# grantjr1842/delayed-streams-modeling

Hardware: AMD Instinct MI355X
Metric: real-time stream throughput, stt-1b-en_fr @ bs=64 per GPU (Mimi encode + LM decode per 80 ms frame) (higher is better)
Workload: dtype bf16 weights + bf16 KV, f32 activations as three exact bf16 pieces, f32 accumulate (v_mfma_f32_16x16x32_bf16); 1 GPU; stt-1b-en_fr batch=64 streaming, ring KV cache full (750 frames), Mimi encode + LM decode HIP path; streams_per_gpu=64, parallelism=replicas x1 (independent stream batches, no per-step collective), streams=encoder stream || 2 LM group stream(s)

## Files before the change

### delayed-streams-modeling_amd/csrc/dsm_engine_api.inc

```

namespace {

template <typename KVT, int HD, int T>
int launch_attn_t(DsmDevice* e, hipStream_t st, float* out, const float* q, const void* k, const void* v,
                  const uint32_t* start_pos, const uint8_t* active, int B, int H, int ctx, int d, const AttnFused& fq) {
  constexpr int UNR = (sizeof(KVT) == 2 && T == 1 && HD == 128) ? 8 : 4;
  size_t lds = sizeof(float) * ((size_t)T * ctx + 4 * T * HD + 16);
  if ((long)B * H >= 2048 && (size_t)2 * ctx * HD * sizeof(KVT) >= (size_t)256 * 1024) lds += e->attn_lds_pad;
  if (lds > 64 * 1024) {
    static size_t allowed = 0;
    if (lds > allowed) {
      HIPCHK(hipFuncSetAttribute(reinterpret_cast<const void*>(&attn_kernel<KVT, HD, T, UNR>), hipFuncAttributeMaxDynamicSharedMemorySize, (int)lds));
      allowed = lds;
    }
  }
  const int tag = e->tag_attn[e->sid(st)];
  if (T == 1 && HD == 64 && ctx <= 32) {
    const int ph = e->prof_begin(tag, st);
    hipLaunchKernelGGL((attn_small_kernel<KVT, 64>), dim3((B * H + 3) / 4), dim3(256), 0, st, out, q, reinterpret_cast<const KVT*>(k),
                       reinterpret_cast<const KVT*>(v), start_pos, active, B * H, H, ctx, d, fq);
    e->prof_end(ph, st);
    HIPCHK(hipGetLastError());
    return 0;
  }
  const int ph = e->prof_begin(tag, st);
  hipLaunchKernelGGL((attn_kernel<KVT, HD, T, UNR>), dim3(B * H), dim3(256), lds, st, out, q, reinterpret_cast<const KVT*>(k),
                     reinterpret_cast<const KVT*>(v), start_pos, active, H, ctx, d, e->dev_ts_slot(tag, e->sid(st), 0), fq);
  e->prof_end(ph, st);
  HIPCHK(hipGetLastError());
  return 0;
}

template <typename KVT>
int launch_attn(DsmDevice* e, hipStream_t st, float* out, const float* q, const void* k, const void* v,
                const uint32_t* start_pos, const uint8_t* active, int B, int H, int hd, int T, int ctx, int d,
                const AttnFused& fq) {
#define DSM_ATTN(HDv, Tv) \
  if (hd == HDv && T == Tv) return launch_attn_t<KVT, HDv, Tv>(e, st, out, q, k, v, start_pos, active, B, H, ctx, d, fq);
  DSM_ATTN(32, 1) DSM_ATTN(64, 1) DSM_ATTN(128, 1) DSM_ATTN(32, 2) DSM_ATTN(64, 2) DSM_ATTN(128, 2)
#undef DSM_ATTN
  e->set_error("unsupported attention shape head_dim=%d T=%d (head_dim must be 32, 64 or 128; T 1 or 2)", hd, T);
  return DSM_ERR_INVALID;
}

int run_norm(DsmDevice* e, hipStream_t st, float* y, const float* x, const float* w, const float* b, int rows, int d,
             int rms) {
  hipLaunchKernelGGL(row_norm_kernel, dim3(rows), dim3(256), 0, st, y, x, w, b, rows, d,
                     rms ? 1e-8f : 1e-5f, rms);
  HIPCHK(hipGetLastError());
  return 0;
}

template <typename WT, typename KVT>
int transformer_forward(DsmDevice* e, hipStream_t st, const TransformerW& w, TransformerState& s, float* x, float* xn,
                        float* q, float* att, float* ff, int B, int T, const uint8_t* d_mask, float* final_out,
                        RowMap final_map, const float* post_norm_w = nullptr, float* post_norm_out = nullptr, int phase = 0,
                        const CaState* ca = nullptr, bool head_done = false) {
  const dsm_transformer_config& c = w.cfg;
  const int d = c.d_model, H = c.num_heads, hd = d / H, M = B * T;
  const float eps = c.norm == 1 ? 1e-8f : 1e-5f;
  if (phase != 2 && !head_done) {
    hipLaunchKernelGGL(kv_builder_kernel, dim3(B), dim3(64), 0, st, s.pos, s.idx, d_mask, s.start_pos, s.widx,
                       c.positional_embedding == 1 ? s.rope_cs : (float*)nullptr, w.inv_freq, B, T, c.context, hd,
                       w.rope_pos_before ? 1 : 0);
    HIPCHK(hipGetLastError());
    if (int rc = run_norm(e, st, xn, x, w.layers[0].n1w, w.layers[0].n1b, M, d, c.norm)) return rc;
  }
  for (int l = 0; l < c.num_layers; ++l) {
    const TLayerW& L = w.layers[l];
    const bool last = (l == c.num_layers - 1);
    AttnFused fq{};
    fq.nt = sizeof(KVT) == 2;
    if (!(phase == 2 && l == 0)) {
      GemmArgs a = base_args(L.in_proj, xn, plain_map(M, d), M);
      a.Y = q;
      a.d = d; a.hd = hd; a.H = H; a.T = T; a.ctx = c.context;
      a.kcache = s.k[l]; a.vcache = s.v[l];
      a.widx = s.widx;
      a.rope_cs = c.positional_embedding == 1 ? s.rope_cs : nullptr;
      a.active = d_mask;
      a.defer_reduce = (T == 1 && L.in_proj.Kpad > DSM_KC && L.in_proj.K % 32 == 0 && e->fuse_qkv) ? 1 : 0;
      if (int rc = launch_gemm_t<WT, KVT, EPI_QKV, 1>(e, st, a, true)) return rc;
      if (a.defer_reduce) {
        const int mtiles = (M + 15) / 16;
        fq.ws = a.ws;
        fq.ld = (long)a.ws_ntiles * 16;
        fq.cstride = (long)mtiles * 16 * fq.ld;
        fq.chunks = (a.Kpad + DSM_KC - 1) / DSM_KC;
        fq.rope_cs = a.rope_cs;
        fq.widx = s.widx;
      }
    }
    if (!(phase == 2 && l == 0))
      if (int rc = launch_attn<KVT>(e, st, att, q, s.k[l], s.v[l], s.start_pos, d_mask, B, H, hd, T, c.context, d, fq)) return rc;
    if (phase == 1) return 0;
    {
      GemmArgs a = base_args(L.out_proj, att, plain_map(M, d), M);
      a.scale = L.ls1;
      a.res = x; a.rmap = plain_map(M, d);
      a.Y = x; a.ymap = plain_map(M, d);
      if (ca) {
        a.norm_w = L.ncw; a.norm_b = L.ncb; a.norm_out = xn; a.norm_eps = w.ca_norm_rms ? 1e-8f : 1e-5f; a.norm_rms = w.ca_norm_rms;
      } else {
        a.norm_w = L.n2w; a.norm_b = L.n2b; a.norm_out = xn; a.norm_eps = eps; a.norm_rms = c.norm;
      }
      if (int rc = gemm_store<WT>(e, st, a)) return rc;
    }
    if (ca) {
      AttnFused none{};
      none.nt = fq.nt;
      {
        GemmArgs a = base_args(L.ca_q, xn, plain_map(M, d), M);
        a.Y = q; a.ymap = plain_map(M, d);
        a.defer_reduce = (T == 1 && a.Kpad > DSM_KC && a.K % 32 == 0 && !a.bias && d % 4 == 0 && e->fuse_qkv) ? 1 : 0;
        if (int rc = gemm_store<WT>(e, st, a)) return rc;
        if (a.defer_reduce) {
          none.ws = a.ws;
          none.ld = (long)a.ws_ntiles * 16;
          none.cstride = (long)((M + 15) / 16) * 16 * none.ld;
          none.chunks = (a.Kpad + DSM_KC - 1) / DSM_KC;
          none.q_only = 1;
        }
      }
      if (int rc = launch_attn<KVT>(e, st, ca->att, q, ca->k[l], ca->v[l], ca->last, ca->act, B, H, hd, T, ca->smax, d, none)) return rc;
      GemmArgs a = base_args(L.ca_out, ca->att, plain_map(M, d), M);
      a.res = x; a.rmap = plain_map(M, d);
      a.Y = x; a.ymap = plain_map(M, d);
      a.norm_w = L.n2w; a.norm_b = L.n2b; a.norm_out = xn; a.norm_eps = eps; a.norm_rms = c.norm;
      if (int rc = gemm_store<WT>(e, st, a)) return rc;
    }
    if (c.gating) {
      GemmArgs a = base_args(L.ff_in, xn, plain_map(M, d), M);
      a.N = w.hidden;
      a.nt_stride = w.hidden;
      a.Y = ff; a.ymap = plain_map(M, w.hidden);
      if (int rc = launch_gemm_t<WT, KVT, EPI_GATE, 2>(e, st, a, true)) return rc;
    } else {
      GemmArgs a = base_args(L.ff_in, xn, plain_map(M, d), M);
      a.act = 1;
      a.Y = ff; a.ymap = plain_map(M, w.hidden);
      if (int rc = gemm_store<WT>(e, st, a)) return rc;
    }
    {
      GemmArgs a = base_args(L.ff_out, ff, plain_map(M, w.hidden), M);
      a.scale = L.ls2;
      a.res = x; a.rmap = plain_map(M, d);
      if (last && final_out) {
        a.Y = final_out; a.ymap = final_map;
      } else {
        a.Y = x; a.ymap = plain_map(M, d);
      }
      if (!last) {
        a.norm_w = w.layers[l + 1].n1w; a.norm_b = w.layers[l + 1].n1b; a.norm_out = xn; a.norm_eps = eps; a.norm_rms = c.norm;
      } else if (post_norm_out) {
        a.norm_w = post_norm_w; a.norm_b = nullptr; a.norm_out = post_norm_out; a.norm_eps = eps; a.norm_rms = c.norm;
      }
      if (int rc = gemm_store<WT>(e, st, a)) return rc;
    }
  }
  return 0;
}

template <typename F>
int with_kv_type(bool kv_bf16, F&& f) {
  return kv_bf16 ? f(uint16_t{}) : f(float{});
}

int fork_groups(DsmDevice* e, hipStream_t st, size_t G) {
  if (G > 1) {
    HIPCHK(hipEventRecord(e->ev_fork, st));
    for (size_t g = 1; g < G; ++g) HIPCHK(hipStreamWaitEvent(e->s_grp[g], e->ev_fork, 0));
  }
  return 0;
}
template <typename F>
int run_groups(DsmDevice* e, hipStream_t st, size_t G, bool serialize, F&& body) {
  for (size_t g = G; g-- > 0;) {
    hipStream_t gs = (g == 0 || serialize) ? st : e->s_grp[g];
    if (int rc = body(g, gs)) return rc;
    if (g > 0) HIPCHK(hipEventRecord(e->ev_grp_done[g], gs));
  }
  return 0;
}
int join_groups(DsmDevice* e, hipStream_t st, size_t G) {
  for (size_t g = 1; g < G; ++g) HIPCHK(hipStreamWaitEvent(st, e->ev_grp_done[g], 0));
  return 0;
}

int mimi_encode_body(dsm_engine* e, int side, hipStream_t st);
int mimi_encode(dsm_engine* e, int side, hipStream_t st) {
  return run_captured(e, *e->g_enc[side], st, (uint64_t)e->sid(st), [&] { return mimi_encode_body(e, side, st); });
}
int mimi_encode_body(dsm_engine* e, int side, hipStream_t st) {
  const MimiW& w = e->mimi_w;
  MimiState& s = e->mimi[side];
  const int B = e->B;
  const RowMap none = plain_map(1, 1);
  e->tag_gemm[e->sid(st)] = DSM_PROF_GEMM_MIMI;
  e->tag_attn[e->sid(st)] = DSM_PROF_ATTN_MIMI;
  bool fused_front = false;
  {
    const MimiW::Stage& s0 = w.stages[0];
    const ConvGeom& c = w.init_conv;
    fused_front = e->fuse_front && c.in_c == 1 && c.k == 7 && c.stride == 1 && c.out_c == 64 && c.S == 6 && !c.lin.bf16 &&
                  s0.ra.k == 3 && s0.ra.stride == 1 && s0.ra.in_c == 64 && s0.ra.out_c == 32 && s0.ra.S == 2 && !s0.ra.lin.bf16 &&
                  s0.rb.k == 1 && s0.rb.stride == 1 && s0.rb.in_c == 32 && s0.rb.out_c == 64 && !s0.rb.lin.bf16 &&
                  c.T_in % 64 == 0 && c.T_out == c.T_in && s0.ra.T_in == c.T_in && s0.rb.T_in == c.T_in && s0.down.in_c == 64 &&
                  s0.down.T_in == c.T_in && !c.replicate && !s0.ra.replicate;
    if (fused_front) {
      SeanetFrontArgs fa;
      fa.cat_init = s.cat_init;
      fa.w0 = reinterpret_cast<const float*>(c.lin.w); fa.b0 = c.lin.bias; fa.ld0 = c.lin.Kpad;
      fa.w1 = reinterpret_cast<const float*>(s0.ra.lin.w); fa.b1 = s0.ra.lin.bias; fa.ld1 = s0.ra.lin.Kpad;
      fa.w2 = reinterpret_cast<const float*>(s0.rb.lin.w); fa.b2 = s0.rb.lin.bias; fa.ld2 = s0.rb.lin.Kpad;
      fa.cat_ra = s.stages[0].cat_ra;
      fa.cat_down = s.stages[0].cat_down;
      fa.T = c.T_in; fa.S0 = c.S; fa.Sd = s0.down.S;
      const int ph = e->prof_begin(e->tag_gemm[e->sid(st)], st);
      hipLaunchKernelGGL(seanet_front_kernel<64>, dim3(c.T_in / 64, B), dim3(256), seanet_front_lds<64>(), st, fa);
      e->prof_end(ph, st);
      HIPCHK(hipGetLastError());
    } else if (int rc = run_conv(e, st, c, s.cat_init, B, s.stages[0].y, plain_map(B * c.T_out, c.out_c), s.stages[0].cat_ra,
                                 cat_map(s0.ra), nullptr, none)) {
      return rc;
    }
  }
  for (size_t i = 0; i < w.stages.size(); ++i) {
    const MimiW::Stage& sw = w.stages[i];
    MimiState::Stage& ss = s.stages[i];
    if (!(i == 0 && fused_front)) {
      if (int rc = run_conv(e, st, sw.ra, ss.cat_ra, B, nullptr, none, ss.cat_rb, cat_map(sw.rb), nullptr, none)) return rc;
      if (int rc = run_conv(e, st, sw.rb, ss.cat_rb, B, nullptr, none, ss.cat_down, cat_map(sw.down), ss.y,
                            plain_map(B * sw.rb.T_out, sw.rb.out_c)))
        return rc;
    }
    if (i + 1 < w.stages.size()) {
      const MimiW::Stage& nx = w.stages[i + 1];
      if (int rc = run_conv(e, st, sw.down, ss.cat_down, B, s.stages[i + 1].y,
                            plain_map(B * sw.down.T_out, sw.down.out_c), s.stages[i + 1].cat_ra, cat_map(nx.ra), nullptr, none))
        return rc;
    } else {
      if (int rc = run_conv(e, st, sw.down, ss.cat_down, B, nullptr, none, s.cat_final, cat_map(w.final_conv), nullptr, none))
        return rc;
    }
  }
  const int Tt = w.final_conv.T_out, d = w.cfg.dimension;
  if (int rc = run_conv(e, st, w.final_conv, s.cat_final, B, s.x_tr, plain_map(B * Tt, d), nullptr, none, nullptr, none))
    return rc;
  if (int rc = transformer_forward<float, float>(e, st, w.tr, s.tr, s.x_tr, s.xn, s.q, s.att, s.ff, B, Tt, s.mask,
                                                  s.cat_ds, cat_map(w.downsample)))
    return rc;
  if (s.first_call && w.downsample.S > 0) {
    hipLaunchKernelGGL(conv_replicate_init_kernel, dim3(B), dim3(256), 0, st, s.h_descs[s.ds_desc]);
    HIPCHK(hipGetLastError());
  }
  if (int rc = run_conv(e, st, w.downsample, s.cat_ds, B, s.latent, plain_map(B, d), nullptr, none, nullptr, none)) return rc;
  const int n_q = w.cfg.quantizer_n_q, qd = w.cfg.quantizer_dim;
  e->tag_gemm[e->sid(st)] = DSM_PROF_RVQ;
  for (int which = 0; which < 2; ++which) {
    const RvqW& r = which == 0 ? w.rvq_first : w.rvq_rest;
    if (r.n_q == 0) continue;
    float* res = which == 0 ? s.res_first : s.res_rest;
    {
// ... 1185 lines not shown
```

### delayed-streams-modeling_amd/csrc/dsm_kernels.h

```cpp
#pragma once
#include <hip/hip_runtime.h>
#include <stdint.h>
#include "dsm_numerics.h"
#include "dsm_sampling.h"

typedef float f32x4 __attribute__((ext_vector_type(4)));
typedef short dsm_bf16x8 __attribute__((ext_vector_type(8)));

__device__ __forceinline__ float wave_sum64(float v) {
#pragma unroll
  for (int off = 32; off >= 1; off >>= 1) v = v + __shfl_xor(v, off, 64);
  return v;
}

enum { EPI_STORE = 0, EPI_QKV = 1, EPI_GATE = 2, EPI_RVQ = 3 };

struct RowMap {
  long bstride;
  int rpb;
  int ld;
  int toff;
  __host__ __device__ long off(int m) const { return (long)(m / rpb) * bstride + (long)((m % rpb) + toff) * ld; }
};

struct GemmArgs {
  const float* X;
  RowMap xmap;
  const void* W;
  int Kpad, K, N, M;
  int nt_stride;
  int wpacked;
  int w_ntiles;
  int wg_cols;
  const float* bias;
  const float* scale;
  const float* res;
  RowMap rmap;
  float* Y;
  RowMap ymap;
  float* Y2;
  RowMap y2map;
  int act;
  int vec;
  int d, hd, H, T, ctx;
  void* kcache;
  void* vcache;
  const uint32_t* widx;
  const float* rope_cs;
  const uint8_t* active;
  float* pval;
  uint32_t* pidx;
  float* ws;
  int ws_ntiles;
  int defer_reduce;
  int chunk_loop;
  const float* norm_w;
  const float* norm_b;
  float* norm_out;
  float norm_eps;
  int norm_rms;
  unsigned long long* ts;
};

template <typename WT>
__device__ __forceinline__ const WT* dsm_wbase(const GemmArgs& a, const WT* W, int n0, int r, int q) {
  if (sizeof(WT) == 2 && a.wpacked) return W + ((long)(n0 >> 4) * (a.Kpad >> 5)) * 512 + (q * 16 + r) * 8;
  return W + (long)(n0 + r) * a.Kpad + 8 * q;
}
template <typename WT>
__device__ __forceinline__ int dsm_wstep(const GemmArgs& a) { return (sizeof(WT) == 2 && a.wpacked) ? 16 : 1; }

__device__ __forceinline__ void launch_stamp_begin(unsigned long long* ts) {
  if (!ts || threadIdx.x != 0) return;
  const unsigned lin = blockIdx.x + gridDim.x * (blockIdx.y + gridDim.y * blockIdx.z);
  if (lin < 128) atomicMin(&ts[0], wall_clock64());
}
__device__ __forceinline__ void launch_stamp_end(unsigned long long* ts) {
  if (!ts || threadIdx.x != 0) return;
  const unsigned total = gridDim.x * gridDim.y * gridDim.z;
  const unsigned lin = blockIdx.x + gridDim.x * (blockIdx.y + gridDim.y * blockIdx.z);
  if (lin + 512 >= total) atomicMax(&ts[1], wall_clock64());
}

template <typename WT>
__device__ __forceinline__ void load_w8(const WT* p, float (&o)[8]);
template <>
__device__ __forceinline__ void load_w8<uint16_t>(const uint16_t* p, float (&o)[8]) {
  uint4 v = *reinterpret_cast<const uint4*>(p);
  o[0] = __uint_as_float(v.x << 16); o[1] = __uint_as_float(v.x & 0xFFFF0000u);
  o[2] = __uint_as_float(v.y << 16); o[3] = __uint_as_float(v.y & 0xFFFF0000u);
  o[4] = __uint_as_float(v.z << 16); o[5] = __uint_as_float(v.z & 0xFFFF0000u);
  o[6] = __uint_as_float(v.w << 16); o[7] = __uint_as_float(v.w & 0xFFFF0000u);
}
template <>
__device__ __forceinline__ void load_w8<float>(const float* p, float (&o)[8]) {
  float4 a = *reinterpret_cast<const float4*>(p);
  float4 b = *reinterpret_cast<const float4*>(p + 4);
  o[0] = a.x; o[1] = a.y; o[2] = a.z; o[3] = a.w; o[4] = b.x; o[5] = b.y; o[6] = b.z; o[7] = b.w;
}

template <typename KVT>
struct Raw8;
typedef unsigned int dsm_u32x4 __attribute__((ext_vector_type(4)));
typedef float dsm_f32x4v __attribute__((ext_vector_type(4)));
template <>
struct Raw8<uint16_t> {
  uint4 v;
  __device__ __forceinline__ void load(const uint16_t* p) { v = *reinterpret_cast<const uint4*>(p); }
  __device__ __forceinline__ void load_nt(const uint16_t* p) {
    const dsm_u32x4 t = __builtin_nontemporal_load(reinterpret_cast<const dsm_u32x4*>(p));
    v = make_uint4(t[0], t[1], t[2], t[3]);
  }
  __device__ __forceinline__ void unpack(float (&o)[8]) const {
    o[0] = __uint_as_float(v.x << 16); o[1] = __uint_as_float(v.x & 0xFFFF0000u);
    o[2] = __uint_as_float(v.y << 16); o[3] = __uint_as_float(v.y & 0xFFFF0000u);
    o[4] = __uint_as_float(v.z << 16); o[5] = __uint_as_float(v.z & 0xFFFF0000u);
    o[6] = __uint_as_float(v.w << 16); o[7] = __uint_as_float(v.w & 0xFFFF0000u);
  }
};
template <>
struct Raw8<float> {
  float4 a, b;
  __device__ __forceinline__ void load(const float* p) {
    a = *reinterpret_cast<const float4*>(p);
    b = *reinterpret_cast<const float4*>(p + 4);
  }
  __device__ __forceinline__ void load_nt(const float* p) {
    const dsm_f32x4v t0 = __builtin_nontemporal_load(reinterpret_cast<const dsm_f32x4v*>(p));
    const dsm_f32x4v t1 = __builtin_nontemporal_load(reinterpret_cast<const dsm_f32x4v*>(p + 4));
    a = make_float4(t0[0], t0[1], t0[2], t0[3]);
    b = make_float4(t1[0], t1[1], t1[2], t1[3]);
  }
  __device__ __forceinline__ void unpack(float (&o)[8]) const {
    o[0] = a.x; o[1] = a.y; o[2] = a.z; o[3] = a.w; o[4] = b.x; o[5] = b.y; o[6] = b.z; o[7] = b.w;
  }
};

__device__ __forceinline__ void store_kv(uint16_t* p, float v) { *p = dsm_f32_to_bf16(v); }
__device__ __forceinline__ void store_kv(float* p, float v) { *p = v; }

__device__ __forceinline__ void store_kv4(uint16_t* p, const float (&o)[4]) {
  uint2 v;
  v.x = (uint32_t)dsm_f32_to_bf16(o[0]) | ((uint32_t)dsm_f32_to_bf16(o[1]) << 16);
  v.y = (uint32_t)dsm_f32_to_bf16(o[2]) | ((uint32_t)dsm_f32_to_bf16(o[3]) << 16);
  *reinterpret_cast<uint2*>(p) = v;
}
__device__ __forceinline__ void store_kv4(float* p, const float (&o)[4]) {
  *reinterpret_cast<float4*>(p) = make_float4(o[0], o[1], o[2], o[3]);
}

template <typename KVT, int EPI>
__device__ __forceinline__ void epi_store_qkv(const GemmArgs& a, f32x4 v, int m, int n) {
  if (m >= a.M || n >= a.N) return;
  const bool full = a.vec && (n + 3 < a.N);
  if (EPI == EPI_STORE) {
    float o[4];
#pragma unroll
    for (int i = 0; i < 4; ++i) {
      float t = v[i];
      if (n + i < a.N) {
        if (a.bias) t = t + a.bias[n + i];
        if (a.act == 1) t = dsm_gelu_erf(t);
        if (a.scale) t = t * a.scale[n + i];
      }
      o[i] = t;
    }
    if (a.res) {
      const float* rp = a.res + a.rmap.off(m) + n;
      if (full) {
        float4 rv = *reinterpret_cast<const float4*>(rp);
        o[0] = rv.x + o[0]; o[1] = rv.y + o[1]; o[2] = rv.z + o[2]; o[3] = rv.w + o[3];
      } else {
#pragma unroll
        for (int i = 0; i < 4; ++i)
          if (n + i < a.N) o[i] = rp[i] + o[i];
      }
    }
    if (a.Y) {
      float* y = a.Y + a.ymap.off(m) + n;
      if (full) {
        *reinterpret_cast<float4*>(y) = make_float4(o[0], o[1], o[2], o[3]);
      } else {
#pragma unroll
        for (int i = 0; i < 4; ++i)
          if (n + i < a.N) y[i] = o[i];
      }
    }
    if (a.Y2) {
      float* y2 = a.Y2 + a.y2map.off(m) + n;
      if (full) {
        *reinterpret_cast<float4*>(y2) = make_float4(dsm_elu(o[0]), dsm_elu(o[1]), dsm_elu(o[2]), dsm_elu(o[3]));
      } else {
#pragma unroll
        for (int i = 0; i < 4; ++i)
          if (n + i < a.N) y2[i] = dsm_elu(o[i]);
      }
    }
  } else {
    const int part = n / a.d, c = n - part * a.d, h = c / a.hd, i0 = c - h * a.hd;
    const int b = m / a.T;
    float o[4] = {v[0], v[1], v[2], v[3]};
    if (part < 2 && a.rope_cs) {
      const float4 cs = *reinterpret_cast<const float4*>(a.rope_cs + ((long)m * (a.hd / 2) + (i0 >> 1)) * 2);
      const float co[2] = {cs.x, cs.z}, si[2] = {cs.y, cs.w};
#pragma unroll
      for (int p = 0; p < 2; ++p) {
        float x0 = v[2 * p], x1 = v[2 * p + 1];
        float t0 = x0 * co[p], t1 = x1 * si[p], t2 = x0 * si[p], t3 = x1 * co[p];
        o[2 * p] = t0 - t1;
        o[2 * p + 1] = t2 + t3;
      }
    }
    if (part == 0) {
      *reinterpret_cast<float4*>(a.Y + (long)m * a.d + c) = make_float4(o[0], o[1], o[2], o[3]);
    } else if (a.active[b]) {
      KVT* cache = reinterpret_cast<KVT*>(part == 1 ? a.kcache : a.vcache);
      store_kv4(cache + (((long)b * a.H + h) * a.ctx + a.widx[m]) * a.hd + i0, o);
    }
  }
}

__device__ __forceinline__ void epi_gate(const GemmArgs& a, f32x4 g, f32x4 u, int m, int n) {
  if (m >= a.M || n >= a.N) return;
  float o[4];
#pragma unroll
  for (int i = 0; i < 4; ++i) o[i] = dsm_silu(g[i]) * u[i];
  float* y = a.Y + a.ymap.off(m) + n;
  if (a.vec && n + 3 < a.N) {
    *reinterpret_cast<float4*>(y) = make_float4(o[0], o[1], o[2], o[3]);
  } else {
#pragma unroll
    for (int i = 0; i < 4; ++i)
      if (n + i < a.N) y[i] = o[i];
  }
}

__device__ __forceinline__ void epi_rvq(const GemmArgs& a, f32x4 v, int m, int n, int tile16, int q) {
  float bv = DSM_INF_F;
  uint32_t bi = 0xFFFFFFFFu;
#pragma unroll
  for (int i = 0; i < 4; ++i) {
    float dist = a.bias[n + i] - v[i];
    if (n + i < a.N && (dist < bv || (dist == bv && (uint32_t)(n + i) < bi))) { bv = dist; bi = (uint32_t)(n + i); }
  }
#pragma unroll
  for (int off = 16; off <= 32; off <<= 1) {
    float ov = __shfl_xor(bv, off, 64);
    uint32_t oi = __shfl_xor(bi, off, 64);
    if (ov < bv || (ov == bv && oi < bi)) { bv = ov; bi = oi; }
  }
  if (q == 0 && m < a.M) {
    a.pval[(long)tile16 * a.M + m] = bv;
    a.pidx[(long)tile16 * a.M + m] = bi;
  }
}

template <typename WT, typename KVT, int MT, int NT, int EPI, bool XALIGNED, bool BX3 = false>
__global__ void gemm_mfma_kernel(GemmArgs a) {
  extern __shared__ __attribute__((aligned(16))) float lds_part[];
  const int lane = threadIdx.x & 63, wave = threadIdx.x >> 6, S = blockDim.x >> 6;
  const int r = lane & 15, q = lane >> 4;
  const int m_base = blockIdx.y * (16 * MT);
  const int n_base = blockIdx.x * ((EPI == EPI_GATE) ? 16 : 16 * NT);
  const WT* W = reinterpret_cast<const WT*>(a.W);
  constexpr int TILES = NT * MT;

  const WT* wrow[NT];
#pragma unroll
  for (int nt = 0; nt < NT; ++nt) wrow[nt] = dsm_wbase<WT>(a, W, n_base + nt * a.nt_stride, r, q);
  const int wst = dsm_wstep<WT>(a);
  const float* xrow[MT];
#pragma unroll
  for (int mt = 0; mt < MT; ++mt) {
    int m = m_base + 16 * mt + r;
    m = m < a.M ? m : a.M - 1;
    xrow[mt] = a.X + a.xmap.off(m) + 8 * q;
  }
  f32x4 acc[NT][MT];
  const int chunks = (a.Kpad + DSM_KC - 1) / DSM_KC;

  for (int c = wave; c < chunks; c += S) {
#pragma unroll
    for (int nt = 0; nt < NT; ++nt)
#pragma unroll
      for (int mt = 0; mt < MT; ++mt) acc[nt][mt] = (f32x4){0.f, 0.f, 0.f, 0.f};
    const int k0 = c * DSM_KC;
    const int k1 = min(k0 + DSM_KC, a.Kpad);
    for (int kb = k0; kb < k1; kb += 32) {
      float wa[NT][8], xb[MT][8];
#pragma unroll
// ... 548 lines not shown
}

#define DSM_ROW_ITS 4

__device__ __forceinline__ void row_norm_apply(const float4 (&v)[DSM_ROW_ITS], float s, float s2, int d, float eps, int rms,
                                               const float* __restrict__ w, const float* __restrict__ b,
                                               float* __restrict__ out) {
  float mm = 1.f, mean = 0.f, inv = 0.f;
  if (rms) {
    mm = sqrtf(s2 / (float)d + eps);
  } else {
    mean = s / (float)d;
    float var = s2 / (float)d - mean * mean;
    inv = 1.0f / sqrtf(var + eps);
  }
#pragma unroll
  for (int it = 0; it < DSM_ROW_ITS; ++it) {
    const int i = it * 1024 + 4 * (int)threadIdx.x;
    if (i < d) {
      const float4 wv = *reinterpret_cast<const float4*>(w + i);
      float4 o;
      if (rms) {
        o.x = (v[it].x / mm) * wv.x; o.y = (v[it].y / mm) * wv.y; o.z = (v[it].z / mm) * wv.z; o.w = (v[it].w / mm) * wv.w;
      } else {
        const float4 bv = *reinterpret_cast<const float4*>(b + i);
        o.x = ((v[it].x - mean) * inv) * wv.x + bv.x; o.y = ((v[it].y - mean) * inv) * wv.y + bv.y;
        o.z = ((v[it].z - mean) * inv) * wv.z + bv.z; o.w = ((v[it].w - mean) * inv) * wv.w + bv.w;
      }
      *reinterpret_cast<float4*>(out + i) = o;
    }
  }
}

template <int ITS>
__global__ __launch_bounds__(256 * ITS) void gemm_reduce_rows_kernel(GemmArgs a, int chunks) {
  constexpr int RS = ITS == 4 ? 16 : 24;
  __shared__ float red[8];
  __shared__ float carry[2][256];
  launch_stamp_begin(a.ts ? a.ts + 2 : nullptr);
  const int m = blockIdx.x;
  const int d = a.N;
  const int it = threadIdx.x >> 8, t = threadIdx.x & 255;
  const long ld = (long)a.ws_ntiles * 16, cstride = (long)((a.M + 15) >> 4) * 16 * ld;
  const int i = it * 1024 + 4 * t;
  const bool live = i < d;
  const float* p = a.ws + (long)m * ld + (live ? i : 4 * t);
  const int ic = live ? i : 4 * t;
  const f32x4 bias4 = *reinterpret_cast<const f32x4*>(a.bias ? a.bias + ic : p);
  const f32x4 scale4 = *reinterpret_cast<const f32x4*>(a.scale ? a.scale + ic : p);
  const f32x4 res4 = *reinterpret_cast<const f32x4*>(a.res ? a.res + a.rmap.off(m) + ic : p);
  const f32x4 nw4 = *reinterpret_cast<const f32x4*>(a.norm_w + ic);
  const f32x4 nb4 = *reinterpret_cast<const f32x4*>(a.norm_rms ? p : a.norm_b + ic);
  f32x4 tot = *reinterpret_cast<const f32x4*>(p);
  for (int c0 = 1; c0 < chunks; c0 += RS) {
    f32x4 w[RS];
#pragma unroll
    for (int u = 0; u < RS; ++u) {
      const int c = c0 + u < chunks ? c0 + u : chunks - 1;
      w[u] = *reinterpret_cast<const f32x4*>(p + c * cstride);
    }
    __builtin_amdgcn_sched_barrier(0);
#pragma unroll
    for (int u = 0; u < RS; ++u)
      if (c0 + u < chunks) tot = tot + w[u];
  }
  float o[4] = {tot[0], tot[1], tot[2], tot[3]};
  if (live) {
#pragma unroll
    for (int j = 0; j < 4; ++j) {
      if (a.bias) o[j] = o[j] + bias4[j];
      if (a.act == 1) o[j] = dsm_gelu_erf(o[j]);
      if (a.scale) o[j] = o[j] * scale4[j];
    }
    if (a.res) {
      o[0] = res4[0] + o[0]; o[1] = res4[1] + o[1]; o[2] = res4[2] + o[2]; o[3] = res4[3] + o[3];
    }
    *reinterpret_cast<float4*>(a.Y + a.ymap.off(m) + i) = make_float4(o[0], o[1], o[2], o[3]);
  }
  float s = 0.0f, s2 = 0.0f;
#pragma unroll
  for (int k = 0; k < ITS; ++k) {
    if (it == k) {
      if (k > 0) { s = carry[0][t]; s2 = carry[1][t]; }
      if (live) {
        s = s + o[0]; s2 = DSM_FMAF(o[0], o[0], s2);
        s = s + o[1]; s2 = DSM_FMAF(o[1], o[1], s2);
        s = s + o[2]; s2 = DSM_FMAF(o[2], o[2], s2);
        s = s + o[3]; s2 = DSM_FMAF(o[3], o[3], s2);
      }
      if (k + 1 < ITS) { carry[0][t] = s; carry[1][t] = s2; }
    }
    if (k + 1 < ITS) __syncthreads();
  }
  if (it == ITS - 1) {
    const int lane = t & 63, wave = t >> 6;
    s = wave_sum64(s);
    s2 = wave_sum64(s2);
    if (lane == 0) { red[wave] = s; red[4 + wave] = s2; }
  }
  __syncthreads();
  s = ((red[0] + red[1]) + red[2]) + red[3];
  s2 = ((red[4] + red[5]) + red[6]) + red[7];
  if (live) {
    float mm = 1.f, mean = 0.f, inv = 0.f;
    if (a.norm_rms) {
      mm = sqrtf(s2 / (float)d + a.norm_eps);
    } else {
      mean = s / (float)d;
      float var = s2 / (float)d - mean * mean;
      inv = 1.0f / sqrtf(var + a.norm_eps);
    }
    float4 r;
    if (a.norm_rms) {
      r.x = (o[0] / mm) * nw4[0]; r.y = (o[1] / mm) * nw4[1]; r.z = (o[2] / mm) * nw4[2]; r.w = (o[3] / mm) * nw4[3];
    } else {
      r.x = ((o[0] - mean) * inv) * nw4[0] + nb4[0]; r.y = ((o[1] - mean) * inv) * nw4[1] + nb4[1];
      r.z = ((o[2] - mean) * inv) * nw4[2] + nb4[2]; r.w = ((o[3] - mean) * inv) * nw4[3] + nb4[3];
    }
    *reinterpret_cast<float4*>(a.norm_out + (long)m * d + i) = r;
  }
  launch_stamp_end(a.ts ? a.ts + 2 : nullptr);
}

__global__ __launch_bounds__(256) void row_norm_kernel(float* __restrict__ y, const float* __restrict__ x,
                                                       const float* __restrict__ w, const float* __restrict__ b, int rows,
                                                       int d, float eps, int rms) {
  __shared__ float red[8];
  const int row = blockIdx.x;
  const float* xr = x + (long)row * d;
  float4 v[DSM_ROW_ITS];
  float s = 0.0f, s2 = 0.0f;
#pragma unroll
  for (int it = 0; it < DSM_ROW_ITS; ++it) {
    const int i = it * 1024 + 4 * (int)threadIdx.x;
    v[it] = make_float4(0.f, 0.f, 0.f, 0.f);
    if (i < d) {
      v[it] = *reinterpret_cast<const float4*>(xr + i);
      s = s + v[it].x; s2 = DSM_FMAF(v[it].x, v[it].x, s2);
      s = s + v[it].y; s2 = DSM_FMAF(v[it].y, v[it].y, s2);
      s = s + v[it].z; s2 = DSM_FMAF(v[it].z, v[it].z, s2);
      s = s + v[it].w; s2 = DSM_FMAF(v[it].w, v[it].w, s2);
    }
  }
  block_row_sums(s, s2, red);
  row_norm_apply(v, s, s2, d, eps, rms, w, b, y + (long)row * d);
}

struct AttnFused {
  const float* ws;
  long ld, cstride;
  int chunks;
  const float* rope_cs;
  const uint32_t* widx;
  int nt;
  int q_only;
};

template <typename KVT, int HD, int T, int UNRB = 8>
__global__ __launch_bounds__(256, 4) void attn_kernel(float* __restrict__ out, const float* __restrict__ qbuf,
                                                   const KVT* __restrict__ kcache, const KVT* __restrict__ vcache,
                                                   const uint32_t* __restrict__ start_pos,
                                                   const uint8_t* __restrict__ active, int H, int ctx, int d,
                                                   unsigned long long* __restrict__ ts, AttnFused fq) {
  constexpr int NW = 4, LPK = HD / 8, G = 64 / LPK;
  extern __shared__ __attribute__((aligned(16))) float lds[];
  const int b = blockIdx.x / H, h = blockIdx.x % H;
  const bool ts_first = ts && threadIdx.x == 0 && blockIdx.x < 256;
  const bool ts_last = ts && threadIdx.x == 0 && blockIdx.x + 1024 >= gridDim.x;
  if (ts_first) atomicMin(&ts[0], wall_clock64());
  if (!active[b]) {
    if (ts_last) atomicMax(&ts[1], wall_clock64());
    return;
  }
  const int tid = threadIdx.x, lane = tid & 63, wave = tid >> 6;
  const int g = lane / LPK, li = lane % LPK;
  float* sc = lds;
  float* red = lds + T * ctx;
  float* scratch = red + NW * T * HD;

  const uint32_t sp = start_pos[b];
  const long e1 = (long)sp + T - 1;
  const int nvalid = (int)((e1 + 1 < (long)ctx) ? e1 + 1 : ctx);
  const float scale = (float)(1.0 / sqrt((double)HD));

  const KVT* Kb = kcache + ((long)b * H + h) * ctx * HD;
  const KVT* Vb = vcache + ((long)b * H + h) * ctx * HD;
  if (T == 1 && fq.ws) {
    if (tid < (fq.q_only ? HD / 4 : 3 * HD / 4)) {
      const int part = tid / (HD / 4), i0 = 4 * (tid % (HD / 4));
      const f32x4 v = slab_sum(fq.ws + (long)b * fq.ld + part * d + h * HD + i0, fq.cstride, fq.chunks);
      float o[4] = {v[0], v[1], v[2], v[3]};
      if (part < 2 && fq.rope_cs) {
        const float4 cs = *reinterpret_cast<const float4*>(fq.rope_cs + ((long)b * (HD / 2) + (i0 >> 1)) * 2);
        const float co[2] = {cs.x, cs.z}, si[2] = {cs.y, cs.w};
#pragma unroll
        for (int p = 0; p < 2; ++p) {
          float x0 = v[2 * p], x1 = v[2 * p + 1];
          float t0 = x0 * co[p], t1 = x1 * si[p], t2 = x0 * si[p], t3 = x1 * co[p];
          o[2 * p] = t0 - t1;
          o[2 * p + 1] = t2 + t3;
        }
      }
      if (part == 0) {
        red[i0] = o[0]; red[i0 + 1] = o[1]; red[i0 + 2] = o[2]; red[i0 + 3] = o[3];
      } else {
        KVT* row = const_cast<KVT*>(part == 1 ? Kb : Vb) + (long)fq.widx[b] * HD + i0;
        store_kv4(row, o);
      }
    }
    __syncthreads();
  }
  float qv[T][8];
#pragma unroll
  for (int t = 0; t < T; ++t) {
    if (T == 1 && fq.ws) {
#pragma unroll
      for (int dd = 0; dd < 8; ++dd) qv[t][dd] = red[8 * li + dd];
    } else {
      const float* qp = qbuf + ((long)(b * T + t)) * d + h * HD + 8 * li;
      float4 q0 = *reinterpret_cast<const float4*>(qp), q1 = *reinterpret_cast<const float4*>(qp + 4);
      qv[t][0] = q0.x; qv[t][1] = q0.y; qv[t][2] = q0.z; qv[t][3] = q0.w;
      qv[t][4] = q1.x; qv[t][5] = q1.y; qv[t][6] = q1.z; qv[t][7] = q1.w;
    }
  }
  if (T == 1 && fq.ws) __syncthreads();

  constexpr int UNR = sizeof(KVT) == 2 ? UNRB : 4;
  constexpr int STEP = UNR * NW * G;
  const int jlast = nvalid - 1;
  const int last_slot = (int)(e1 % ctx);
  Raw8<KVT> ra[UNR], rb[UNR];
#define DSM_ISSUE(R, BASE, J0)                                                        \
  _Pragma("unroll") for (int u = 0; u < UNR; ++u) {                                    \
    const int jj = min((J0) + u * NW * G + g, jlast);                                  \
    if (fq.nt) R[u].load_nt(BASE + (long)jj * HD + 8 * li);                            \
    else R[u].load(BASE + (long)jj * HD + 8 * li);                                     \
  }
#define DSM_SCORES(R, J0)                                                              \
  _Pragma("unroll") for (int u = 0; u < UNR; ++u) {                                    \
    const int j = (J0) + u * NW * G + g;                                               \
    int delta = last_slot - min(j, jlast);  \
    delta += (delta < 0) ? ctx : 0;                                                    \
    float kv[8];                                                                       \
    R[u].unpack(kv);                                                                   \
    _Pragma("unroll") for (int t = 0; t < T; ++t) {                                    \
      float p = 0.0f;                                                                  \
      _Pragma("unroll") for (int dd = 0; dd < 8; ++dd) p = DSM_FMAF(qv[t][dd], kv[dd], p); \
      _Pragma("unroll") for (int off = LPK / 2; off >= 1; off >>= 1) p = p + __shfl_xor(p, off, 64); \
      if (li == 0 && j < nvalid) sc[t * ctx + j] = (delta >= T - 1 - t) ? p * scale : -DSM_INF_F; \
    }                                                                                  \
  }
  {
    int j0 = wave * G;
    DSM_ISSUE(ra, Kb, j0)
    while (j0 < nvalid) {
      DSM_ISSUE(rb, Kb, j0 + STEP)
      DSM_SCORES(ra, j0)
      j0 += STEP;
      if (j0 >= nvalid) break;
      DSM_ISSUE(ra, Kb, j0 + STEP)
      DSM_SCORES(rb, j0)
      j0 += STEP;
    }
  }
  DSM_ISSUE(ra, Vb, wave * G)
  __syncthreads();

  float lsum[T];
#pragma unroll
  for (int t = 0; t < T; ++t) {
    float m = -DSM_INF_F;
    for (int j = tid; j < nvalid; j += 256) m = fmaxf(m, sc[t * ctx + j]);
#pragma unroll
    for (int off = 32; off >= 1; off >>= 1) m = fmaxf(m, __shfl_xor(m, off, 64));
    if (lane == 0) scratch[wave] = m;
    __syncthreads();
    m = fmaxf(fmaxf(scratch[0], scratch[1]), fmaxf(scratch[2], scratch[3]));
    __syncthreads();
    float tp = 0.0f;
    for (int j = tid; j < nvalid; j += 256) {
      float p = dsm_expf(sc[t * ctx + j] - m);
      sc[t * ctx + j] = p;
      tp = tp + p;
    }
    tp = wave_sum64(tp);
    if (lane == 0) scratch[4 + wave] = tp;
    __syncthreads();
    lsum[t] = ((scratch[4] + scratch[5]) + scratch[6]) + scratch[7];
    __syncthreads();
  }

  float acc[T][8];
#pragma unroll
  for (int t = 0; t < T; ++t)
#pragma unroll
    for (int dd = 0; dd < 8; ++dd) acc[t][dd] = 0.0f;
#define DSM_PV(R, J0)                                                                  \
  _Pragma("unroll") for (int u = 0; u < UNR; ++u) {  \
    const int j = (J0) + u * NW * G + g;                                               \
    float vv[8];                                                                       \
    R[u].unpack(vv);                                                                   \
    _Pragma("unroll") for (int t = 0; t < T; ++t) {                                    \
       \
      const float wgt = (j < nvalid) ? sc[t * ctx + j] / lsum[t] : 0.0f;               \
      _Pragma("unroll") for (int dd = 0; dd < 8; ++dd) acc[t][dd] = DSM_FMAF(wgt, vv[dd], acc[t][dd]); \
    }                                                                                  \
  }
  {
    int j0 = wave * G;
    while (j0 < nvalid) {
      DSM_ISSUE(rb, Vb, j0 + STEP)
      DSM_PV(ra, j0)
      j0 += STEP;
      if (j0 >= nvalid) break;
      DSM_ISSUE(ra, Vb, j0 + STEP)
      DSM_PV(rb, j0)
      j0 += STEP;
    }
  }
#undef DSM_ISSUE
#undef DSM_SCORES
#undef DSM_PV
#pragma unroll
  for (int t = 0; t < T; ++t)
#pragma unroll
    for (int dd = 0; dd < 8; ++dd) {
      float v = acc[t][dd];
#pragma unroll
      for (int off = 32; off >= LPK; off >>= 1) v = v + __shfl_xor(v, off, 64);
      acc[t][dd] = v;
    }
  if (g == 0) {
#pragma unroll
    for (int t = 0; t < T; ++t)
#pragma unroll
      for (int dd = 0; dd < 8; ++dd) red[(wave * T + t) * HD + 8 * li + dd] = acc[t][dd];
  }
  __syncthreads();
  for (int i = tid; i < T * HD; i += 256) {
    int t = i / HD, dd = i % HD;
    float tot = ((red[(0 * T + t) * HD + dd] + red[(1 * T + t) * HD + dd]) + red[(2 * T + t) * HD + dd]) +
                red[(3 * T + t) * HD + dd];
    out[((long)(b * T + t)) * d + h * HD + dd] = tot;
  }
  if (ts_last) atomicMax(&ts[1], wall_clock64());
}

template <typename KVT, int HD>
__global__ __launch_bounds__(256) void attn_small_kernel(float* __restrict__ out, const float* __restrict__ qbuf,
                                                         const KVT* __restrict__ kcache, const KVT* __restrict__ vcache,
                                                         const uint32_t* __restrict__ start_pos, const uint8_t* __restrict__ active,
                                                         int BH, int H, int ctx, int d, AttnFused fq) {
  static_assert(HD == 64, "one lane group of 8 lanes per key");
  constexpr int LPK = HD / 8;
  __shared__ __attribute__((aligned(16))) float lds_all[4][32 + HD];
  const int tid = threadIdx.x, lane = tid & 63, wave = tid >> 6;
  const int unit = blockIdx.x * 4 + wave;
  const int uc = unit < BH ? unit : BH - 1;
  const int b = uc / H, h = uc % H;
  const bool on = unit < BH && active[b];
  float* sc = lds_all[wave];
  float* qs = sc + 32;
  const int g = lane / LPK, li = lane % LPK;
  const uint32_t sp = start_pos[b];
  const long e1 = (long)sp;
  const int nvalid = (int)((e1 + 1 < (long)ctx) ? e1 + 1 : ctx);
  const float scale = (float)(1.0 / sqrt((double)HD));
  const KVT* Kb = kcache + ((long)b * H + h) * ctx * HD;
  const KVT* Vb = vcache + ((long)b * H + h) * ctx * HD;
  if (fq.ws) {
    if (on && lane < (fq.q_only ? HD / 4 : 3 * HD / 4)) {
      const int part = lane / (HD / 4), i0 = 4 * (lane % (HD / 4));
      const f32x4 v = slab_sum(fq.ws + (long)b * fq.ld + part * d + h * HD + i0, fq.cstride, fq.chunks);
      float o[4] = {v[0], v[1], v[2], v[3]};
      if (part < 2 && fq.rope_cs) {
        const float4 cs = *reinterpret_cast<const float4*>(fq.rope_cs + ((long)b * (HD / 2) + (i0 >> 1)) * 2);
        const float co[2] = {cs.x, cs.z}, si[2] = {cs.y, cs.w};
#pragma unroll
        for (int p = 0; p < 2; ++p) {
          float x0 = v[2 * p], x1 = v[2 * p + 1];
          float t0 = x0 * co[p], t1 = x1 * si[p], t2 = x0 * si[p], t3 = x1 * co[p];
          o[2 * p] = t0 - t1;
          o[2 * p + 1] = t2 + t3;
        }
      }
      if (part == 0) {
        qs[i0] = o[0]; qs[i0 + 1] = o[1]; qs[i0 + 2] = o[2]; qs[i0 + 3] = o[3];
      } else {
        KVT* row = const_cast<KVT*>(part == 1 ? Kb : Vb) + (long)fq.widx[b] * HD + i0;
        store_kv4(row, o);
      }
    }
    __syncthreads();
  }
  if (!on) return;
  float qv[8];
  if (fq.ws) {
#pragma unroll
    for (int dd = 0; dd < 8; ++dd) qv[dd] = qs[8 * li + dd];
  } else {
    const float* qp = qbuf + (long)b * d + h * HD + 8 * li;
    const float4 q0 = *reinterpret_cast<const float4*>(qp), q1 = *reinterpret_cast<const float4*>(qp + 4);
    qv[0] = q0.x; qv[1] = q0.y; qv[2] = q0.z; qv[3] = q0.w; qv[4] = q1.x; qv[5] = q1.y; qv[6] = q1.z; qv[7] = q1.w;
  }
  const int jlast = nvalid - 1;
  Raw8<KVT> rk[4], rv[4];
#pragma unroll
  for (int w = 0; w < 4; ++w) {
    const int jj = min(8 * w + g, jlast);
    rk[w].load(Kb + (long)jj * HD + 8 * li);
  }
#pragma unroll
  for (int w = 0; w < 4; ++w) {
    const int jj = min(8 * w + g, jlast);
    rv[w].load(Vb + (long)jj * HD + 8 * li);
  }
#pragma unroll
  for (int w = 0; w < 4; ++w) {
    const int j = 8 * w + g;
    float kv[8];
    rk[w].unpack(kv);
    float p = 0.0f;
#pragma unroll
    for (int dd = 0; dd < 8; ++dd) p = DSM_FMAF(qv[dd], kv[dd], p);
#pragma unroll
    for (int off = LPK / 2; off >= 1; off >>= 1) p = p + __shfl_xor(p, off, 64);
    if (li == 0 && j < nvalid) sc[j] = p * scale;
  }
  float m = -DSM_INF_F;
  if (lane < nvalid) m = fmaxf(m, sc[lane]);
#pragma unroll
  for (int off = 32; off >= 1; off >>= 1) m = fmaxf(m, __shfl_xor(m, off, 64));
  float tp = 0.0f;
  if (lane < nvalid) {
    const float p = dsm_expf(sc[lane] - m);
    sc[lane] = p;
    tp = tp + p;
  }
  tp = wave_sum64(tp);
  const float lsum = ((tp + 0.0f) + 0.0f) + 0.0f;
  float tot[8];
#pragma unroll
  for (int w = 0; w < 4; ++w) {
    const int j = 8 * w + g;
    float vv[8];
    rv[w].unpack(vv);
    const float wgt = (j < nvalid) ? sc[j] / lsum : 0.0f;
#pragma unroll
    for (int dd = 0; dd < 8; ++dd) {
      float v = (j < nvalid) ? DSM_FMAF(wgt, vv[dd], 0.0f) : 0.0f;
#pragma unroll
      for (int off = 32; off >= LPK; off >>= 1) v = v + __shfl_xor(v, off, 64);
      tot[dd] = w == 0 ? v : tot[dd] + v;
    }
  }
  if (g == 0) {
    float* o = out + (long)b * d + h * HD + 8 * li;
    *reinterpret_cast<float4*>(o) = make_float4(tot[0], tot[1], tot[2], tot[3]);
    *reinterpret_cast<float4*>(o + 4) = make_float4(tot[4], tot[5], tot[6], tot[7]);
  }
}

__global__ void kv_builder_kernel(uint32_t* __restrict__ pos, uint32_t* __restrict__ idx,
                                  const uint8_t* __restrict__ active, uint32_t* __restrict__ start_pos,
                                  uint32_t* __restrict__ widx, float* __restrict__ rope_cs,
                                  const float* __restrict__ inv_freq, int B, int T, int ctx, int hd,
                                  int rope_before) {
  const int b = blockIdx.x;
  if (b >= B) return;
  __shared__ uint32_t s_pos_after;
// ... 920 lines not shown
```

Before: 1823 x realtime (stream-seconds of audio per wall second).

## Restructure attention kernel loads, batch score shuffles, and pre-normalize softmax weights

The attention kernel now picks nontemporal KV loads at compile time from the KV type instead of a runtime flag, and computes addresses with 32-bit offsets. Score shuffle reductions are batched across all unrolled keys to expose more instruction-level parallelism. Softmax probabilities are divided by the row sum once in LDS rather than inside the PV loop. The V prefetch is issued two steps ahead so the first PV iterations overlap memory latency. This adds register pressure and an extra LDS pass, and the 32-bit offset math overflows if a cache grows too large.

```diff
diff --git a/delayed-streams-modeling_amd/csrc/dsm_engine_api.inc b/delayed-streams-modeling_amd/csrc/dsm_engine_api.inc
--- a/delayed-streams-modeling_amd/csrc/dsm_engine_api.inc
+++ b/delayed-streams-modeling_amd/csrc/dsm_engine_api.inc
@@ -70,7 +70,6 @@
     const TLayerW& L = w.layers[l];
     const bool last = (l == c.num_layers - 1);
     AttnFused fq{};
-    fq.nt = sizeof(KVT) == 2;
     if (!(phase == 2 && l == 0)) {
       GemmArgs a = base_args(L.in_proj, xn, plain_map(M, d), M);
       a.Y = q;
@@ -108,7 +107,6 @@
     }
     if (ca) {
       AttnFused none{};
-      none.nt = fq.nt;
       {
         GemmArgs a = base_args(L.ca_q, xn, plain_map(M, d), M);
         a.Y = q; a.ymap = plain_map(M, d);
diff --git a/delayed-streams-modeling_amd/csrc/dsm_kernels.h b/delayed-streams-modeling_amd/csrc/dsm_kernels.h
--- a/delayed-streams-modeling_amd/csrc/dsm_kernels.h
+++ b/delayed-streams-modeling_amd/csrc/dsm_kernels.h
@@ -136,6 +136,11 @@
   }
 };
 
+template <typename KVT>
+__device__ __forceinline__ const KVT* kv_at(const KVT* base, int elem) {
+  return reinterpret_cast<const KVT*>(reinterpret_cast<const char*>(base) + (unsigned)(elem * (int)sizeof(KVT)));
+}
+
 __device__ __forceinline__ void store_kv(uint16_t* p, float v) { *p = dsm_f32_to_bf16(v); }
 __device__ __forceinline__ void store_kv(float* p, float v) { *p = v; }
 
@@ -990,7 +995,6 @@
   int chunks;
   const float* rope_cs;
   const uint32_t* widx;
-  int nt;
   int q_only;
 };
 
@@ -1071,21 +1075,33 @@
 #define DSM_ISSUE(R, BASE, J0)                                                        \
   _Pragma("unroll") for (int u = 0; u < UNR; ++u) {                                    \
     const int jj = min((J0) + u * NW * G + g, jlast);                                  \
-    if (fq.nt) R[u].load_nt(BASE + (long)jj * HD + 8 * li);                            \
-    else R[u].load(BASE + (long)jj * HD + 8 * li);                                     \
+    if constexpr (sizeof(KVT) == 2) R[u].load_nt(kv_at(BASE, jj * HD + 8 * li));       \
+    else R[u].load(kv_at(BASE, jj * HD + 8 * li));                                     \
   }
 #define DSM_SCORES(R, J0)                                                              \
-  _Pragma("unroll") for (int u = 0; u < UNR; ++u) {                                    \
-    const int j = (J0) + u * NW * G + g;                                               \
-    int delta = last_slot - min(j, jlast);  \
-    delta += (delta < 0) ? ctx : 0;                                                    \
-    float kv[8];                                                                       \
-    R[u].unpack(kv);                                                                   \
-    _Pragma("unroll") for (int t = 0; t < T; ++t) {                                    \
-      float p = 0.0f;                                                                  \
-      _Pragma("unroll") for (int dd = 0; dd < 8; ++dd) p = DSM_FMAF(qv[t][dd], kv[dd], p); \
-      _Pragma("unroll") for (int off = LPK / 2; off >= 1; off >>= 1) p = p + __shfl_xor(p, off, 64); \
-      if (li == 0 && j < nvalid) sc[t * ctx + j] = (delta >= T - 1 - t) ? p * scale : -DSM_INF_F; \
+  {                                                                                    \
+    float p[UNR][T];                                                                   \
+    _Pragma("unroll") for (int u = 0; u < UNR; ++u) {                                  \
+      float kv[8];                                                                     \
+      R[u].unpack(kv);                                                                 \
+      _Pragma("unroll") for (int t = 0; t < T; ++t) {                                  \
+        p[u][t] = 0.0f;                                                                \
+        _Pragma("unroll") for (int dd = 0; dd < 8; ++dd) p[u][t] = DSM_FMAF(qv[t][dd], kv[dd], p[u][t]); \
+      }                                                                                \
+    }                                                                                  \
+    _Pragma("unroll") for (int off = LPK / 2; off >= 1; off >>= 1) {                   \
+      float o[UNR][T];                                                                 \
+      _Pragma("unroll") for (int u = 0; u < UNR; ++u)                                  \
+        _Pragma("unroll") for (int t = 0; t < T; ++t) o[u][t] = __shfl_xor(p[u][t], off, 64); \
+      _Pragma("unroll") for (int u = 0; u < UNR; ++u)                                  \
+        _Pragma("unroll") for (int t = 0; t < T; ++t) p[u][t] = p[u][t] + o[u][t];     \
+    }                                                                                  \
+    _Pragma("unroll") for (int u = 0; u < UNR; ++u) {                                  \
+      const int j = (J0) + u * NW * G + g;                                             \
+      int delta = last_slot - min(j, jlast);  \
+      delta += (delta < 0) ? ctx : 0;                                                  \
+      _Pragma("unroll") for (int t = 0; t < T; ++t)                                    \
+        if (li == 0 && j < nvalid) sc[t * ctx + j] = (delta >= T - 1 - t) ? p[u][t] * scale : -DSM_INF_F; \
     }                                                                                  \
   }
   {
@@ -1102,6 +1118,7 @@
     }
   }
   DSM_ISSUE(ra, Vb, wave * G)
+  DSM_ISSUE(rb, Vb, wave * G + STEP)
   __syncthreads();
 
   float lsum[T];
@@ -1125,6 +1142,7 @@
     if (lane == 0) scratch[4 + wave] = tp;
     __syncthreads();
     lsum[t] = ((scratch[4] + scratch[5]) + scratch[6]) + scratch[7];
+    for (int j = tid; j < nvalid; j += 256) sc[t * ctx + j] = sc[t * ctx + j] / lsum[t];
     __syncthreads();
   }
 
@@ -1140,20 +1158,21 @@
     R[u].unpack(vv);                                                                   \
     _Pragma("unroll") for (int t = 0; t < T; ++t) {                                    \
        \
-      const float wgt = (j < nvalid) ? sc[t * ctx + j] / lsum[t] : 0.0f;               \
+      const float wgt = (j < nvalid) ? sc[t * ctx + j] : 0.0f;                         \
       _Pragma("unroll") for (int dd = 0; dd < 8; ++dd) acc[t][dd] = DSM_FMAF(wgt, vv[dd], acc[t][dd]); \
     }                                                                                  \
   }
   {
     int j0 = wave * G;
     while (j0 < nvalid) {
-      DSM_ISSUE(rb, Vb, j0 + STEP)
       DSM_PV(ra, j0)
       j0 += STEP;
       if (j0 >= nvalid) break;
       DSM_ISSUE(ra, Vb, j0 + STEP)
       DSM_PV(rb, j0)
       j0 += STEP;
+      if (j0 >= nvalid) break;
+      DSM_ISSUE(rb, Vb, j0 + STEP)
     }
   }
 #undef DSM_ISSUE
```

New measurement: 1770 x realtime (stream-seconds of audio per wall second). 0.971x the previous value.
